# NyanCAD/Cadnip.jl

Measured on AMD Instinct MI355X. Metric: newton_iters_per_sec, higher is better.
Workload: dtype f64; 1 GPU; gf180 DFF transient 0-700 ns (synthetic sp_mos1 level-1 card, 30 MOSFETs, n=235, nnz=1090), 4096 Vdd x temp corner instances per GPU (state resident in HBM; one 8-instance workgroup per CU in flight, the rest handed out by the kernel's instance queue); step = DC init + full transient of the batch; instances_per_gpu=4096, instances_total=4096, fused=2, newton_mode=1, launches_last_step=5120, accepted_last_step=6078488, rejected_last_step=692364

## Files before the change

### cadnip.jl_amd/csrc/devices.hpp

```cpp
#pragma once
#include <hip/hip_runtime.h>
#include <math.h>
#include "../../include/cadnip_hip.h"

namespace cadnip {

#define CADNIP_CHARGE_SCALE 1e12

#ifdef CADNIP_TRACE
static __device__ unsigned long long g_trace_sum[64], g_trace_cnt[64];
static __device__ int g_trace_wave;
__shared__ unsigned long long g_trace_last;
#define CADNIP_TRACE_FINE(id) (((id) >= 8 && (id) <= 15) || (id) >= 20 || (id) == 0 || (id) == 2)
#define CADNIP_TRACE_POINT(id)                                                                          \
  do {                                                                                                  \
    if ((CADNIP_TRACE + 0 >= 2 || !CADNIP_TRACE_FINE(id)) && blockIdx.x == 0 && (int)(threadIdx.x >> 6) == g_trace_wave) { \
      unsigned long long _t = clock64();                                                                \
      if ((threadIdx.x & 63) == 0) {                                                                    \
        atomicAdd(&g_trace_sum[id], _t - g_trace_last); atomicAdd(&g_trace_cnt[id], 1ull); g_trace_last = _t; \
      }                                                                                                 \
    }                                                                                                   \
  } while (0)
#elif defined(CADNIP_MARKS)
#define CADNIP_TRACE_POINT(id) asm volatile("; @@MARK " #id)
#else
#define CADNIP_TRACE_POINT(id) do {} while (0)
#endif

__device__ __forceinline__ double dpp_pair_swap(double v) {
  int lo = __double2loint(v), hi = __double2hiint(v);
  lo = __builtin_amdgcn_update_dpp(0, lo, 0xB1, 0xF, 0xF, false);
  hi = __builtin_amdgcn_update_dpp(0, hi, 0xB1, 0xF, 0xF, false);
  return __hiloint2double(hi, lo);
}

template <class NodeT> struct DevCtxT {
  const NodeT* __restrict__ nodes;
  const int* __restrict__ ipar;
  const double* __restrict__ par;
  const double* __restrict__ wave;
  int count;
  int dev;
  double t;
  int mode;
  int initjct;
  const double* __restrict__ cache = nullptr;
};
typedef DevCtxT<int> DevCtx;

struct SlotOut {
  static constexpr bool DIRECT = false;
  __device__ __forceinline__ void Rn(int, double) const {}
  __device__ __forceinline__ double du(int) const { return 0.0; }
  double* __restrict__ g;
  double* __restrict__ c;
  double* __restrict__ b;
  int count, dev;
  __device__ __forceinline__ void G(int k, double v) const { g[k * count + dev] = v; }
  __device__ __forceinline__ void C(int k, double v) const { c[k * count + dev] = v; }
// ... 644 lines not shown
  CADNIP_TRACE_POINT(27);
}


__device__ __forceinline__ D3 m1_swap_pair(const D3& x) {
  D3 r;
  r.v = dpp_pair_swap(x.v);
#pragma unroll
  for (int i = 0; i < 3; ++i) r.p[i] = dpp_pair_swap(x.p[i]);
  return r;
}
__device__ __forceinline__ D3 m1_sel(bool c, const D3& x, const D3& y) {
  D3 r;
  r.v = c ? x.v : y.v;
#pragma unroll
  for (int i = 0; i < 3; ++i) r.p[i] = c ? x.p[i] : y.p[i];
  return r;
}


template <class Ctx, class Out>
__device__ inline void stamp_mos1_pair(const Ctx& d, const double* u, const Out& s, double* limit_w_base, int side, bool valid) {
  const double CS = CADNIP_CHARGE_SCALE;
  const bool D = side != 0;
  int nd = node_of(d, 0), ng = node_of(d, 1), ns = node_of(d, 2), nb = node_of(d, 3), ndi = node_of(d, 4), nsi = node_of(d, 5);
  int l0 = node_of(d, 6), l1 = node_of(d, 7), l2 = node_of(d, 8), l3 = node_of(d, 9);
  double Vd = volt(u, nd), Vg = volt(u, ng), Vs = volt(u, ns), Vb = volt(u, nb), Vdi = volt(u, ndi), Vsi = volt(u, nsi);
  double type = par_of(d, M1_TYPE), vt = par_of(d, M1_VT), tPhi = par_of(d, M1_TPHI), tVbi = par_of(d, M1_TVBI);
  double gamma = par_of(d, M1_GAMMA);
  const double mf = par_of(d, M1_MFACTOR), gmin_p = par_of(d, M1_GMIN), isat = par_of(d, D ? M1_DSATCUR : M1_SSATCUR);
  const double lambda = par_of(d, M1_LAMBDA), Beta = par_of(d, M1_BETA);
  const int vdep = Out::DIRECT ? d.ipar[d.dev] : 0;
  __builtin_amdgcn_sched_barrier(0);
  CADNIP_TRACE_POINT(20);
  double w_gs, w_ds, w_bs, w_bd;
  m1_limit(d, u, type, vt, tPhi, tVbi, gamma, Vg, Vb, Vdi, Vsi, l0, l1, l2, l3, w_gs, w_ds, w_bs, w_bd);
  if (limit_w_base && valid && !D) { limit_w_base[l0] = w_gs; limit_w_base[l1] = w_ds; limit_w_base[l2] = w_bs; limit_w_base[l3] = w_bd; }
  CADNIP_TRACE_POINT(21);
  {
    const double gl[6] = {1.0, -1.0, 1.0, 1.0, -1.0, 1.0};
    s.Gv(6 * side, gl);
    if constexpr (Out::DIRECT) {
      s.Rn(D ? l2 : l0, u[D ? l2 : l0] - ((D ? Vb : Vg) - Vsi));
      s.Rn(D ? l3 : l1, u[D ? l3 : l1] - (D ? Vb - Vdi : Vdi - Vsi));
    }
  }
  CADNIP_TRACE_POINT(22);
  D3 a = D3::seed(type * w_gs, 0), b = D3::seed(type * w_ds, 1), c = D3::seed(type * w_bs, 2);
  D3 dvbd = c - b, dvgd = a - b;
  const D3 vj = m1_sel(D, dvbd, c);
  const double gmin_m = gmin_p / mf;
  const double q_cb = par_of(d, D ? M1_CBD : M1_CBS), q_cbsw = par_of(d, D ? M1_CBDSW : M1_CBSSW), q_pot = par_of(d, M1_TBULKPOT), q_dep = par_of(d, M1_TDEPCAP);
  const double q_mj = par_of(d, M1_MJ), q_mjsw = par_of(d, M1_MJSW), q_f2 = par_of(d, D ? M1_F2D : M1_F2S), q_f3 = par_of(d, D ? M1_F3D : M1_F3S), q_f4 = par_of(d, D ? M1_F4D : M1_F4S);
  __builtin_amdgcn_sched_barrier(0);
  const D3 cj = m1_junction(vj, vt, gmin_m, isat), co = m1_swap_pair(cj);
  const D3 cbs = m1_sel(D, co, cj), cbd = m1_sel(D, cj, co);
  CADNIP_TRACE_POINT(23);
  int mode;
  D3 dvon, vdsat, cdrain;
  m1_channel(a, b, c, dvbd, dvgd, tPhi, tVbi, type, gamma, lambda, Beta, mode, dvon, vdsat, cdrain);
  CADNIP_TRACE_POINT(24);
  const D3 cdreq = (mode >= 0 ? type : -type) * cdrain;
  const double dW_gs = (Vg - Vsi) - w_gs, dW_ds = (Vdi - Vsi) - w_ds, dW_bs = (Vb - Vsi) - w_bs;
  const double Vk[6] = {Vd, Vg, Vs, Vb, Vdi, Vsi};
  auto row = [&](const D3& I, double (&g)[6], double& Ieq) {
    const double fa = type * I.p[0], fb = type * I.p[1], fc = type * I.p[2];
// ... 194 lines not shown
```

### cadnip.jl_amd/csrc/fused2.hip

```cpp
#include <hip/hip_runtime.h>
#include <stdio.h>
#include <stdlib.h>
#include <string.h>
#include <algorithm>
#include <vector>
#include "fused_team_kernel.hpp"

namespace cadnip {

struct F2Tables {
  std::vector<unsigned> data;
  int off[S_NSEC];
  void begin(int which) { if (data.size() & 1) data.push_back(0); off[which] = (int)data.size(); }
  void add16(const std::vector<int>& v) {
    for (size_t i = 0; i < v.size(); i += 2) data.push_back((unsigned)(v[i] & 0xFFFF) | ((i + 1 < v.size() ? (unsigned)(v[i + 1] & 0xFFFF) : 0u) << 16));
  }
  void add32(unsigned x) { data.push_back(x); }
  void add64(u64 x) { data.push_back((unsigned)x); data.push_back((unsigned)(x >> 32)); }
};

template <class Build>
static void upload_steps(StepList& L, int lu_words, Build&& build) {
  if (L.d) (void)hipFree(L.d);
  L = StepList();
// ... 109 lines not shown
}

int fused2_tables(CadnipHandle* h) {
  FusedState& S = h->f2;
  if (!h->analyzed) return CADNIP_NOTREADY;
  if (S.d_tab && !S.dirty) return CADNIP_OK;
  S.release();
  F2Tables T;
  if (!f2_prepare(h, T)) return CADNIP_BADARG;
  HIP_TRY(hipMalloc((void**)&S.d_tab, T.data.size() * sizeof(unsigned)));
  HIP_TRY(hipMemcpy(S.d_tab, T.data.data(), T.data.size() * sizeof(unsigned), hipMemcpyHostToDevice));
  for (int i = 0; i < S_NSEC; ++i) S.off[i] = T.off[i];
  S.dirty = false;
  return CADNIP_OK;
}

static int fused2_blocks(CadnipHandle* h) {
  { int rc = fused2_tables(h); if (rc) return rc; }
  FusedState& S = h->f2;
  if (S.blk_dirty || !S.d_blk) {
    F2Block hb[F2_MAX_BLOCKS];
    int nb = 0;
    for (size_t bi = 0; bi < h->blocks.size() && nb < F2_MAX_BLOCKS; ++bi) {
      auto& b = h->blocks[bi];
      if (b.count == 0) continue;
      hb[nb++] = F2Block{b.d_ipar, b.d_par, b.type, b.count, b.n_par, b.g_base, b.c_base, b.b_base, S.nodes_off[bi], b.mos1_plain ? 1 : 0, -1};
    }
    for (int i = 0; i < nb; ++i)
      for (int j = i + 1; j < nb; ++j)
        if ((hb[j].type == CADNIP_DEV_MOS1) > (hb[i].type == CADNIP_DEV_MOS1)) { F2Block tmp = hb[i]; hb[i] = hb[j]; hb[j] = tmp; }
    auto first_of = [&](int ta, int tb) { for (int i = 0; i < nb; ++i) if (hb[i].type == ta || hb[i].type == tb) return i; return -1; };
    S.rc_blk = first_of(CADNIP_DEV_CAPACITOR, CADNIP_DEV_RESISTOR);
    S.src_blk = first_of(CADNIP_DEV_VSOURCE, CADNIP_DEV_ISOURCE);
    S.lean = true;
    for (int i = 0; i < nb; ++i) {
      const int ty = hb[i].type;
      const bool heavy = ty == CADNIP_DEV_DIODE || ty == CADNIP_DEV_DIODECAP || ty == CADNIP_DEV_SIMPLEMOS || ty == CADNIP_DEV_BVSOURCE ||
                         ty == CADNIP_DEV_BISOURCE || ty == CADNIP_DEV_VA || (ty == CADNIP_DEV_MOS1 && !hb[i].mos1_plain);
      if (heavy) S.lean = false;
    }
    if (!S.steps1.d || lds_bytes(lds_sweep((size_t)0, S.lean_end - S.lean_lo, S.steps1.len, S.lu_words, h->n, 0, 8)) > LDS_BUDGET) S.lean = false;
    S.n_blk = nb;
    S.par_words = 0;
    { bool first = true;
      for (int i = 0; i < nb; ++i)
        if (hb[i].type == CADNIP_DEV_MOS1 && hb[i].mos1_plain) {
          if (!first || hb[i].count > 32) { hb[i].lds_par = S.par_words; S.par_words += hb[i].n_par * hb[i].count; }
          first = false;
        } }
    if (!S.d_blk) HIP_TRY(hipMalloc((void**)&S.d_blk, sizeof(hb)));
    HIP_TRY(hipStreamSynchronize(h->stream));
    HIP_TRY(hipMemcpy(S.d_blk, hb, sizeof(F2Block) * (size_t)nb, hipMemcpyHostToDevice));
    S.blk_dirty = false;
  }
  return CADNIP_OK;
}

F2Plan fused2_plan(CadnipHandle* h, F2Mode mode, int newton_mode) {
  F2Plan p;
  FusedState& S = h->f2;
  p.rc = CADNIP_BADARG;
  if (h->va_ext || !h->analyzed) return p;
  if (fused2_tables(h)) return p;
  int nb = 0;
  for (auto& b : h->blocks) nb += b.count > 0;
  if (nb > F2_MAX_BLOCKS || lds_bytes(lds_sweep((size_t)0, S.full_len, 0, S.lu_words, h->n, 0, 1)) > LDS_BUDGET) return p;
  if (int rc = fused2_blocks(h)) { p.rc = rc; return p; }
  const bool direct = !getenv("CADNIP_F2_NODIRECT"), lean = direct && S.lean;
  p.keep_factors = mode != F2_DC && (newton_mode || mode == F2_STEP);
  if (p.keep_factors && !lean) return p;
  p.circuit_ok = true;
  if (h->homotopy || h->spec.gshunt != 0.0 || h->spec.srcFact < 1.0) return p;
  if (S.n_cu <= 0) {
    int cu = 0;
    if (hipError_t e = hipDeviceGetAttribute(&cu, hipDeviceAttributeMultiprocessorCount, h->device)) { set_last_error("hipDeviceGetAttribute", e); p.rc = CADNIP_HIPERROR; return p; }
    S.n_cu = cu > 0 ? cu : 256;
  }
  p.var = !direct ? 2 : S.lean ? 0 : 1;
  p.tab_len = S.full_len;
  if (lean) { p.tab_lo = S.lean_lo; p.tab_len = S.lean_end - S.lean_lo; }
  if (mode != F2_DC && lean) {
    int nw = h->B <= S.n_cu ? 4 : h->B <= 2 * S.n_cu ? 2 : 0;
    if (const char* e = getenv("CADNIP_F2_TEAM")) nw = atoi(e) >= 4 ? 4 : atoi(e) >= 2 ? 2 : 0;
    if (mode == F2_STEP) nw = 4;
    const StepList& T = S.team[nw / 4];
    const size_t shmem = lds_bytes(lds_team((size_t)0, p.tab_len, nw ? T.len : 0, S.lu_words, h->n, S.par_words, nw));
    if (nw && T.d && shmem <= LDS_BUDGET) {
      const int wg_per_cu = (int)std::max<size_t>(1, std::min<size_t>(LDS_BUDGET / shmem, (size_t)(16 / nw)));
      p.nw = nw; p.steps = &T; p.shmem = shmem; p.grid = std::min(h->B, S.n_cu * wg_per_cu); p.rc = CADNIP_OK;
      return p;
    }
  }
  if (mode == F2_STEP) return p;
  if (lean) p.steps = &S.steps1;
  auto bytes = [&](int wpb) { return lds_bytes(lds_sweep((size_t)0, p.tab_len, p.steps ? p.steps->len : 0, S.lu_words, h->n, 0, wpb)); };
  int wpb = 8;
  if (const char* e = getenv("CADNIP_F2_WPB")) wpb = atoi(e) >= 8 ? 8 : atoi(e) >= 4 ? 4 : atoi(e) >= 2 ? 2 : 1;
  while (wpb > 1 && (bytes(wpb) > LDS_BUDGET || S.n_cu * (wpb / 2) >= h->B)) wpb >>= 1;
  if (bytes(wpb) > LDS_BUDGET) return p;
  const int wg_per_cu = (int)std::max<size_t>(1, std::min<size_t>(LDS_BUDGET / bytes(wpb), (size_t)(32 / wpb)));
  size_t shmem = bytes(wpb);
  if (p.steps && lds_steps_predec_ok(S.lu_words, h->n) && !getenv("CADNIP_F2_STEPS_PACKED")) {
    const size_t pd = lds_bytes(lds_sweep((size_t)0, p.tab_len, lds_sweep_desc_words(p.steps->len, true), S.lu_words, h->n, 0, wpb));
    if (pd <= LDS_BUDGET && (int)std::max<size_t>(1, std::min<size_t>(LDS_BUDGET / pd, (size_t)(32 / wpb))) == wg_per_cu) { p.step_predec = true; shmem = pd; }
  }
  p.wpb = wpb; p.shmem = shmem; p.grid = std::min((h->B + wpb - 1) / wpb, S.n_cu * wg_per_cu); p.rc = CADNIP_OK;
  return p;
}

static int launch_fused2(CadnipHandle* h, const TranArgs& t, int rounds, const F2DcOpts* dc, const F2StepOpts* step = nullptr) {
  const F2Plan p = fused2_plan(h, dc ? F2_DC : step ? F2_STEP : F2_TRAN, t.newton_mode);
  if (p.rc) return p.rc;
  ProfScope ps(h, dc ? "fused2_dc" : step ? "fused_step" : "fused2_newton");
  FusedState& S = h->f2;
  F2Args f{};
  f.n_blk = S.n_blk; f.rc_blk = S.rc_blk; f.src_blk = S.src_blk;
  f.blk = (const F2Block*)S.d_blk;
  f.wave = h->d_wave;
  f.tab = S.d_tab;
  for (int i = 0; i < S_NSEC; ++i) f.off[i] = S.off[i];
  f.tab_len = p.tab_len; f.tab_lo = p.tab_lo;
  f.n = h->n; f.nnz = h->nnz; f.nnz_lu = S.lu_words;
  f.n_pre = S.n_pre; f.n_post = S.n_post; f.nc = S.nc; f.dn0 = S.dn0; f.n_fwd = S.n_fwd;
  if (p.steps) { f.team_desc = p.steps->d; f.team_desc_len = p.steps->len; f.ts_pre = p.steps->n_steps[0]; f.ts_post = p.steps->n_steps[1]; f.ts_fwd = p.steps->n_steps[2]; }
  f.step_predec = p.step_predec ? 1 : 0;
  f.step_refresh = step ? step->refresh : 0; f.step_resid = step ? step->resid : nullptr; f.step_norm = step ? step->norm : nullptr;
  f.step_reps = step ? step->reps : 1; f.step_skip = step ? step->skip : 0;
  if (p.keep_factors) {
    const size_t need = (size_t)h->B * S.lu_words;
    if (need > S.lufac_cap) {
      if (S.d_lufac) (void)hipFree(S.d_lufac);
      S.d_lufac = nullptr; S.lufac_cap = 0;
      HIP_TRY(hipMalloc((void**)&S.d_lufac, need * sizeof(double)));
      S.lufac_cap = need;
    }
    f.lufac = S.d_lufac;
  }
  f.rounds = rounds; f.B = h->B; f.t = t; f.cold = h->d_cold;
  f.dc_mode = 1;
  if (dc) { f.dc_abstol = dc->abstol; f.dc_maxiters = dc->maxiters; f.dc_pcnr = dc->use_pcnr; f.dc_mode = dc->mode; f.dc_initjct = dc->initjct; f.dcstate = dc->dcstate; }
  if (!S.d_queue) HIP_TRY(hipMalloc((void**)&S.d_queue, sizeof(int)));
  TRY_RC(dev_zero_async(h, S.d_queue, sizeof(int)));
  f.queue = S.d_queue;
  const bool debug = getenv("CADNIP_F2_DEBUG") != nullptr;
  if (p.nw) {
    f.par_words = S.par_words;
    if (debug) fprintf(stderr, "[cadnip f2] team of %d waves: B %d n_cu %d grid %d shmem %zu rounds %d nc %d steps %d+%d / %d\n", p.nw, h->B, S.n_cu, p.grid, p.shmem, rounds, S.nc, f.ts_pre, f.ts_post, f.ts_fwd);
    if (step) TRY_RC(fteam_launch_step(std::min(h->B, S.n_cu), p.shmem, h->stream, f));
    else TRY_RC(fteam_launch(p.nw, p.grid, p.shmem, h->stream, f));
  } else {
    const size_t tab_b = (size_t)p.tab_len / 2 * 8, desc_b = (size_t)lds_sweep_desc_words(f.team_desc_len, p.step_predec) * 8;
    if (debug) fprintf(stderr, "[cadnip f2] B %d n_cu %d wpb %d grid %d shmem %zu (tables %zu, steps %zu, per instance %zu) rounds %d nc %d passes %d+%d steps %d+%d / %d (%s) variant %d\n", h->B, S.n_cu, p.wpb, p.grid, p.shmem, tab_b, desc_b, (p.shmem - tab_b - desc_b) / p.wpb, rounds, S.nc, S.n_pre, S.n_post, f.ts_pre, f.ts_post, f.ts_fwd, p.step_predec ? "pre-decoded" : "packed", p.var);
    TRY_RC(p.var == 0 ? f2_launch_variant<0>(p.wpb, dc != nullptr, p.grid, p.shmem, h->stream, f)
         : p.var == 1 ? f2_launch_variant<1>(p.wpb, dc != nullptr, p.grid, p.shmem, h->stream, f)
                      : f2_launch_variant<2>(p.wpb, dc != nullptr, p.grid, p.shmem, h->stream, f));
  }
  HIP_TRY(hipGetLastError());
  return CADNIP_OK;
}

int launch_fused2_rounds(CadnipHandle* h, const TranArgs& t, int rounds) { return launch_fused2(h, t, rounds, nullptr); }

int launch_fused_step(CadnipHandle* h, int refresh, const FusedStepIO& io) {
  TranArgs t;
  memset(&t, 0, sizeof(t));
  t.u = (double*)io.u; t.du = (double*)io.du; t.delta = io.delta; t.limit_w = h->d_limit_w; t.tcur = (double*)io.t; t.gamma = (double*)io.gamma; t.active = h->d_active; t.flags = io.flags;
  t.t = io.t_keep; t.h = io.gamma_keep;
  t.B = h->B; t.n = h->n; t.n_limits = h->n_limits;
  F2StepOpts so{refresh, io.resid, io.norm, io.reps > 0 ? io.reps : 1, io.skip};
  return launch_fused2(h, t, 1 << 30, nullptr, &so);
}

int launch_fused2_dc(CadnipHandle* h, const TranArgs& t, int rounds, double abstol, int maxiters, int use_pcnr, int mode, int initjct, int* d_dcstate) {
  F2DcOpts dc{abstol, maxiters, use_pcnr, mode, initjct, d_dcstate};
  return launch_fused2(h, t, rounds, &dc);
}

}
```

### cadnip.jl_amd/csrc/fused2_kernel.hpp

```cpp
#pragma once
#include <hip/hip_runtime.h>
#include "devices.hpp"
#include "internal.hpp"
#include "tran_ctrl.hpp"
#include "lds_layout.hpp"

namespace cadnip {

typedef unsigned short u16;
typedef unsigned long long u64;
#define NOPOS 0xFFFFu
#define F2_NCMAX 16
#define F2_JU 18
#define F2_MAX_BLOCKS 32

enum { S_GPOS = 0, S_CDESC, S_BROW, S_NZ, S_ENT, S_TERM, S_LEV, S_QINV, S_NODES, S_ROWOF, S_LOADPOS, S_NSEC };

struct F2Block {
  const int* ipar; const double* par;
  int type, count, n_par, g_base, c_base, b_base, nodes_off, mos1_plain;
  int lds_par;
};

typedef const __attribute__((address_space(4))) F2Block* F2BlockPtr;

__device__ __forceinline__ F2Block load_block(const F2Block* blk, int i) {
  F2BlockPtr q = (F2BlockPtr)blk + i;
  F2Block b;
  b.ipar = q->ipar; b.par = q->par; b.type = q->type; b.count = q->count; b.n_par = q->n_par; b.g_base = q->g_base; b.c_base = q->c_base;
  b.b_base = q->b_base; b.nodes_off = q->nodes_off; b.mos1_plain = q->mos1_plain; b.lds_par = q->lds_par;
  return b;
}

struct F2Args {
  const F2Block* blk;
  int n_blk, rc_blk;
  int src_blk;
  const double* wave;
  const unsigned* tab;
  int off[S_NSEC];
  int tab_len;
  int tab_lo;
  int n, nnz, nnz_lu, rounds, B;
  int n_pre, n_post, nc, dn0;
  int n_fwd;
  double* lufac;
  const unsigned long long* team_desc; int team_desc_len;
  int ts_pre, ts_post, ts_fwd;
  int step_predec;
  int par_words;
  int step_refresh; double *step_resid, *step_norm;
  int step_reps, step_skip;
  double dc_abstol; int dc_maxiters, dc_pcnr, dc_mode, dc_initjct; int* dcstate;
  const int* cold;
  int* queue;
  TranArgs t;
};

typedef const __attribute__((address_space(4))) F2Args* F2ArgsK;
__device__ __forceinline__ F2ArgsK kargs() {
  F2ArgsK p = (F2ArgsK)__builtin_amdgcn_kernarg_segment_ptr();
  asm volatile("" : "+s"(p));
  return p;
}
struct TranStateView {
  double *t, *h, *hprev, *hpp, *tcur, *gamma;
  int *nhist, *order, *k, *status, *bp_idx, *save_idx, *active;
  long long* cnt;
  const double *breaks, *save_t;
  int n_break, n_save;
  int newton_mode; double *mn_a0f, *mn_ss, *mn_dnp; int* mn_flags;
  int max_order; double* hp3;
};
__device__ __forceinline__ TranStateView state_view() {
  const F2ArgsK p = kargs();
  TranStateView v;
  v.t = p->t.t; v.h = p->t.h; v.hprev = p->t.hprev; v.hpp = p->t.hpp; v.tcur = p->t.tcur; v.gamma = p->t.gamma;
  v.nhist = p->t.nhist; v.order = p->t.order; v.k = p->t.k; v.status = p->t.status; v.bp_idx = p->t.bp_idx; v.save_idx = p->t.save_idx;
  v.active = p->t.active; v.cnt = p->t.cnt; v.breaks = p->t.breaks; v.save_t = p->t.save_t; v.n_break = p->t.n_break; v.n_save = p->t.n_save;
  v.newton_mode = p->t.newton_mode; v.mn_a0f = p->t.mn_a0f; v.mn_ss = p->t.mn_ss; v.mn_dnp = p->t.mn_dnp; v.mn_flags = p->t.mn_flags;
  v.max_order = p->t.max_order; v.hp3 = p->t.hp3;
  return v;
// ... 194 lines not shown
#pragma unroll
      for (int j = k + 1; j < NC; ++j) A[j] = fma(-m, readlane_f64(A[j], k), A[j]);
      if (lane > k) A[k] = m;
    }
    bc = fma(-m, readlane_f64(bc, k), bc);
  }
#pragma unroll
  for (int k = NC - 1; k >= 0; --k) {
    const double xk = readlane_f64(bc * rp[k], k);
    bc = lane == k ? xk : (lane < k ? fma(-A[k], xk, bc) : bc);
  }
  if (lane < NC) {
    W[yc0 + lane] = bc;
    if (MODE == 0 && keep) {
#pragma unroll
      for (int j = 0; j < NC; ++j) S[j] = j == lane ? rp[j] : A[j];
    }
  }
}

template <int WPB, bool DC, int VAR>
__global__ void __launch_bounds__(64 * WPB) k_fused2(F2Args f) {
  constexpr bool DIRECT = VAR != 2, LEAN = VAR == 0;
  extern __shared__ double sm[];
  const int tid = threadIdx.x, lane0 = tid & 63, w = __builtin_amdgcn_readfirstlane(tid >> 6), n = f.n;
  {
    const uint2* src = (const uint2*)(f.tab + f.tab_lo);
    uint2* dst = (uint2*)sm;
    for (int i = tid; i < f.tab_len / 2; i += 64 * WPB) dst[i] = src[i];
  }
  const TranArgs& a = f.t;
  const unsigned* tab = (const unsigned*)sm;
  const bool predec = LEAN && f.step_predec;
  const LdsSweep<double*> L = lds_sweep((double*)sm, f.tab_len, LEAN ? lds_sweep_desc_words(f.team_desc_len, predec) : 0, f.nnz_lu, n, w, WPB);
  const uint4* tdesc = (const uint4*)L.desc;
  const unsigned char* tflag = (const unsigned char*)(L.desc + (LEAN ? f.team_desc_len : 0));
  if constexpr (LEAN) {
    if (predec) {
      const uint4* src = (const uint4*)f.team_desc;
      uint4* dst = (uint4*)L.desc;
      unsigned char* fl = (unsigned char*)(L.desc + f.team_desc_len);
      for (int i = tid; i < f.team_desc_len / 2; i += 64 * WPB) {
        const uint4 d = src[i];
        const StepPredec p = lds_step_predecode(d.x, d.y, d.z, d.w, (unsigned)(f.nnz_lu + n + lane0));
        dst[i] = make_uint4(p.x, p.y, p.z, p.w);
        fl[i] = (unsigned char)p.flags;
      }
    } else {
      const uint2* src = (const uint2*)f.team_desc;
      uint2* dst = (uint2*)L.desc;
      for (int i = tid; i < f.team_desc_len; i += 64 * WPB) dst[i] = src[i];
    }
  }
  __syncthreads();
  const int nW = L.nW;
  double* W = L.W;
  double* us = L.u;
  double* betas = L.beta;
  if (lane0 == 0) { W[nW] = 0.0; W[nW + 1] = 1.0; }
  const int tlo = f.tab_lo;
  const u16* gpos = (const u16*)(tab + (f.off[S_GPOS] - tlo));
  const u64* cdesc = (const u64*)(tab + (f.off[S_CDESC] - tlo));
  const u16* brow = (const u16*)(tab + (f.off[S_BROW] - tlo));
  const u64* nzd = (const u64*)(tab + (LEAN ? 0 : f.off[S_NZ]));
  const u64* laned = (const u64*)(tab + (LEAN ? 0 : f.off[S_ENT]));
  const unsigned* term = tab + (LEAN ? 0 : f.off[S_TERM]);
  typedef const __attribute__((address_space(4))) u64* PassPtr;
// ... 56 lines not shown
  while (inst < f.B) {
    const TranStateView sv = state_view();
    if (DC) st.status = __builtin_amdgcn_readfirstlane(sv.status[inst]);
    else { st = load_state(sv, inst); make_uniform(st); }
    if (st.status == 0) { have = true; break; }
    int nx = 0;
    if (lane0 == 0) nx = atomicAdd(kargs()->queue, 1);
    inst = (int)gridDim.x * WPB + __builtin_amdgcn_readfirstlane(nx);
  }
  if (!have || budget <= 0) break;
  const size_t vo = (size_t)inst * n;
  double* lw = (DC ? f.dc_pcnr : a.use_pcnr) ? kargs()->t.limit_w + vo : nullptr;
  FusedVecs vec{us, betas, W, qinv, vo, lw};
  if (!DC) vec.load_history(n, lane0);
  {
    const F2ArgsK ka = kargs();
    const double *ug = ka->t.u + vo, *betag = ka->t.beta + vo;
    for (int i = lane0; i < n; i += 64) { us[i] = ug[i]; betas[i] = DC ? 0.0 : betag[i]; }
  }
  const bool mn = !DC && LEAN && a.newton_mode != 0;
  if (mn && (st.mflags & MN_VALID)) {
    const double* src = kargs()->lufac + (size_t)inst * f.nnz_lu;
    for (int i = lane0; i < f.nnz_lu; i += 64) W[i] = src[i];
  }
  int dc_state = 0, dc_iters = 0, dc_first = 0;
  if (DC) { dc_state = __builtin_amdgcn_readfirstlane(kargs()->dcstate[inst]); dc_first = f.dc_initjct && __builtin_amdgcn_readfirstlane(kargs()->cold[inst]); }
  double rc_val[2] = {0.0, 0.0};
  if (f.rc_blk >= 0) {
    const F2Block B = load_block(f.blk, f.rc_blk);
    const double* par = B.par + (size_t)inst * B.n_par * B.count;
#pragma unroll
    for (int q = 0; q < 2; ++q) { const int dev = lane0 + 64 * q; rc_val[q] = par[dev < B.count ? dev : 0]; }
  }
  double src_val = 0.0, src_t = 0.0;
  bool src_have = false;
  int src_seg = 0;
  for (; budget > 0; --budget) {
    int lane = lane0;
    asm volatile("" : "+v"(lane));
    CADNIP_TRACE_POINT(17);
    bool refresh = true;
    if (mn) {
      refresh = (st.mflags & MN_NEED) || !(st.mflags & MN_VALID) ||
                (st.k == 0 && (st.a0 < 0.6 * st.a0f || st.a0 * 0.6 > st.a0f || (st.mflags >> MN_SINCE_SHIFT) >= 20));
      if (refresh) { st.a0f = st.a0; st.ss = 20.0; st.mflags = MN_VALID | MN_JCUR; st.dsc = 1.0; }
      else st.dsc = st.a0 == st.a0f ? 1.0 : fast_div(2.0, 1.0 + fast_div(st.a0, st.a0f));
    }
    if (refresh) {
      for (int i = lane; i < (nW >> 1); i += 64) ((double2*)W)[i] = make_double2(0.0, 0.0);
    } else {
      for (int i = f.nnz_lu + lane; i < nW; i += 64) W[i] = 0.0;
    }
    CADNIP_WAVE_SYNC();
    CADNIP_TRACE_POINT(0);
    const double tcur = DC ? 0.0 : st.tn, a0 = DC ? 0.0 : st.a0;
    const int dmode = DC ? f.dc_mode : 1, dinit = DC ? dc_first : 0;
    const unsigned trash_w = (unsigned)(f.nnz_lu + n + lane);
    dc_first = 0;
    if constexpr (DIRECT) {
      auto at = [&](unsigned nd16) -> double { const double x = us[nd16 == 0xFFFFu ? 0u : nd16]; return nd16 == 0xFFFFu ? 0.0 : x; };
      auto dat = [&](unsigned nd16) -> double {
        const unsigned i = nd16 == 0xFFFFu ? 0u : nd16;
        const double x = a0 * us[i] + betas[i];
        return nd16 == 0xFFFFu ? 0.0 : x;
      };
      if (f.rc_blk >= 0) {
        const bool cap = rc_type == CADNIP_DEV_CAPACITOR;
        double jv[2], cur[2];
#pragma unroll
        for (int q = 0; q < 2; ++q) {
          const unsigned np = rc_nd[q] & 0xFFFFu, nn = rc_nd[q] >> 16;
          const double xp = cap ? dat(np) : at(np), xn = cap ? dat(nn) : at(nn);
          jv[q] = cap ? a0 * rc_val[q] : rc_val[q];
          cur[q] = rc_val[q] * (xp - xn);
        }
#pragma unroll
        for (int q = 0; q < 2; ++q) {
          if (q == 1 && rc_count <= 64) break;
          if (refresh) {
            atomicAdd(&W[rc_gp[q][0] & 0xFFFFu], jv[q]); atomicAdd(&W[rc_gp[q][0] >> 16], -jv[q]);
            atomicAdd(&W[rc_gp[q][1] & 0xFFFFu], -jv[q]); atomicAdd(&W[rc_gp[q][1] >> 16], jv[q]);
          }
          atomicAdd(&W[rc_row[q] & 0xFFFFu], cur[q]); atomicAdd(&W[rc_row[q] >> 16], -cur[q]);
        }
      }
      if (f.src_blk >= 0) {
        if (DC || !src_have || tcur != src_t) {
          const F2Block B = load_block(f.blk, f.src_blk);
          const double* par = B.par + (size_t)inst * B.n_par * B.count;
          LdsCtx d{nodes + B.nodes_off, B.ipar, par, f.wave, B.count, lane < B.count ? lane : 0, tcur, dmode, dinit};
          src_val = source_value(d, par_of(d, 0), par_of(d, 1), &src_seg);
          src_t = tcur; src_have = true;
        }
        if (src_type == CADNIP_DEV_VSOURCE) {
          const double ui = at(src_nd[1]), vd = at(src_nd[0] & 0xFFFFu) - at(src_nd[0] >> 16) - src_val;
          if (refresh) {
            atomicAdd(&W[src_gp[0] & 0xFFFFu], 1.0); atomicAdd(&W[src_gp[0] >> 16], -1.0);
            atomicAdd(&W[src_gp[1] & 0xFFFFu], 1.0); atomicAdd(&W[src_gp[1] >> 16], -1.0);
          }
          atomicAdd(&W[src_row[0] & 0xFFFFu], ui); atomicAdd(&W[src_row[0] >> 16], -ui);
          atomicAdd(&W[src_row[1]], vd);
        } else {
          atomicAdd(&W[src_row[0] & 0xFFFFu], -src_val); atomicAdd(&W[src_row[0] >> 16], src_val);
        }
      }
      CADNIP_TRACE_POINT(13);
    }
    for (int bi = 0; bi < f.n_blk; ++bi) {
      if (DIRECT && ((bi == f.rc_blk && rc_count <= 128) || (bi == f.src_blk && src_count <= 64))) continue;
      const F2Block B = load_block(f.blk, bi);
      const double* par = B.par + (size_t)inst * B.n_par * B.count;
      int dev0 = lane;
      if (DIRECT && bi == f.rc_blk) dev0 = lane + 128;
      if (DIRECT && bi == f.src_blk) dev0 = lane + 64;
      if (!DIRECT && bi == f.rc_blk) {
#pragma unroll
        for (int q = 0; q < 2; ++q) {
          const int dev = lane + 64 * q;
          if (dev < B.count) {
            AccumOutT<false, DIRECT> s{W, betas, a0, gpos + B.g_base, cdesc + B.c_base, brow + B.b_base, B.count, dev, 0u, us, rowof, trash_w};
            if (B.type == CADNIP_DEV_CAPACITOR) capacitance4(s, 0, rc_val[q]); else conductance4(s, 0, rc_val[q]);
            if (DIRECT) {
              const short* nd = nodes + B.nodes_off;
              const int np = nd[dev], nn = nd[B.count + dev];
              residual2(s, np, nn, B.type == CADNIP_DEV_CAPACITOR ? rc_val[q] * (s.du(np) - s.du(nn)) : rc_val[q] * (volt(us, np) - volt(us, nn)));
            }
// ... 287 lines not shown
```

### cadnip.jl_amd/csrc/internal.hpp

```cpp
#pragma once
#include <hip/hip_runtime.h>
#include <stdint.h>
#include <string>
#include <vector>
#include "../../include/cadnip_hip.h"
#include "stamp_plan.hpp"
#include "ac_hbm_plan.hpp"
#define CADNIP_MOS1_PAR_OXCAP 8
#define CADNIP_MOS1_PAR_GD 30
#define CADNIP_MOS1_PAR_GS 31

#define HIP_TRY(expr)                                                     \
  do {                                                                    \
    hipError_t _e = (expr);                                               \
    if (_e != hipSuccess) {                                               \
      cadnip::set_last_error(#expr, _e);                                  \
      return CADNIP_HIPERROR;                                             \
    }                                                                     \
  } while (0)

namespace cadnip {

void set_last_error(const char* what, hipError_t e);

// ... 43 lines not shown
  int type, count, n_nodes, n_ipar, n_par;
  int g_base, c_base, b_base, n_g, n_c, n_b;
  int* d_nodes = nullptr;
  std::vector<int> h_nodes;
  double* d_cache = nullptr; int n_cache = 0;
  int va_model = -1;
  int va_tl = 0;
  bool mos1_plain = false;
  int* d_ipar = nullptr;
  double* d_par = nullptr;
  int sp_cs = 0, sp_chunks = 0;
  struct PlanSet { StampShape shape; int *tptr = nullptr, *info = nullptr; uint4* rec = nullptr; unsigned short* rowoff = nullptr; };
  PlanSet plan[2];
};

struct ProfEntry { const char* name; double ms = 0; int64_t calls = 0; };

struct StepList { unsigned long long* d = nullptr; int len = 0, n_steps[3] = {0, 0, 0}; };

struct FusedState {
  bool dirty = true, blk_dirty = true;
  unsigned int* d_tab = nullptr;
  int off[16] = {0};
  int lu_len = 0;
  int lean_lo = 0, lean_end = 0;
  int full_len = 0;
  int lu_words = 0, nc = 0, dn0 = 0, n_pre = 0, n_post = 0, n_fwd = 0;
  std::vector<int> nodes_off;
  StepList steps1;
  StepList steps4;
  StepList team[2];
  void* d_blk = nullptr;
  int n_blk = 0, rc_blk = -1, src_blk = -1;
  int par_words = 0;
  bool lean = false;
  int* d_queue = nullptr;
  double* d_lufac = nullptr; size_t lufac_cap = 0;
  int n_cu = 0;
  int n_cu_hint() const { return n_cu > 0 ? n_cu : 256; }
  void release();
};

struct AcState {
  bool dirty = true;
  int *d_piv_rows = nullptr, *d_piv_lev_ptr = nullptr;
  unsigned char* d_nodiag = nullptr;
  double *d_bac = nullptr, *d_omega = nullptr, *d_x = nullptr, *d_berr = nullptr;
  int* d_flags = nullptr;
  size_t cap_freq = 0, cap_sys = 0;
  bool adj_ready = false;
  int *d_t_colptr = nullptr, *d_t_pos = nullptr, *d_t_row = nullptr, *d_t_diag = nullptr;
  int *d_ut_rows = nullptr, *d_ut_lev_ptr = nullptr, *d_lt_rows = nullptr, *d_lt_lev_ptr = nullptr;
  int *d_a_colptr = nullptr, *d_a_row = nullptr, *d_a_pos = nullptr;
  int n_ut_lev = 0, n_lt_lev = 0;
  int* d_pairs = nullptr;
  double *d_h = nullptr, *d_adj_x = nullptr, *d_adj_berr = nullptr;
  int* d_adj_flags = nullptr;
  size_t cap_pairs = 0, cap_adj_sys = 0, cap_adj_x = 0;
  double *d_multi_rhs = nullptr, *d_multi_h = nullptr, *d_multi_x = nullptr, *d_multi_berr = nullptr;
  int *d_multi_pairs = nullptr, *d_multi_flags = nullptr;
  size_t cap_multi_rhs = 0, cap_multi_h = 0, cap_multi_x = 0, cap_multi_pairs = 0, cap_multi_cols = 0;
  template <class F> void each_multi_buffer(F f) {
    f((void**)&d_multi_rhs); f((void**)&d_multi_h); f((void**)&d_multi_x); f((void**)&d_multi_berr); f((void**)&d_multi_pairs); f((void**)&d_multi_flags);
  }
  int memory = CADNIP_AC_LDS, max_waves = 0;
  double* d_work = nullptr; size_t cap_work = 0;
// ... 88 lines not shown
};
AcLaunch ac_launch_plan(CadnipHandle* h, long n_sys, int wpb_req);
int ac_lu_prepare(CadnipHandle* h, bool adjoint = false);
int launch_ac_lu(CadnipHandle* h, const AcLaunch& p, int n_freq, long s0, int n_sys, double gmin);
int launch_ac_adjoint(CadnipHandle* h, const AcLaunch& p, int n_freq, long s0, int n_sys, double gmin, int n_pairs, bool want_x);
int launch_ac_multi(CadnipHandle* h, const AcLaunch& p, int n_freq, long s0, int n_sys, double gmin, int n_rhs, int n_pairs, bool want_x);
int launch_ac_adjoint_multi(CadnipHandle* h, const AcLaunch& p, int n_freq, long s0, int n_sys, double gmin, int n_rhs, int n_pairs, bool want_x);
int upload_homotopy(CadnipHandle* h, const double* gshunt , const double* srcfact );
int restore_masks(CadnipHandle* h, bool cold);
int launch_calib_copy(CadnipHandle* h, long n, int reps);
#define TRY_RC(x) do { int _rc_ = (x); if (_rc_) return _rc_; } while (0)
struct MultiCopy { struct Seg { unsigned* dst; const unsigned* src; size_t words; }; Seg seg[8]; int n = 0;
  void add(void* dst, const void* src, size_t bytes) { seg[n].dst = (unsigned*)dst; seg[n].src = (const unsigned*)src; seg[n].words = bytes / 4; ++n; } };
int dev_multi_async(CadnipHandle* h, const MultiCopy& m, bool to_host);
int launch_norm2(CadnipHandle* h, const double* d_x, double* d_out);
int dev_zero_async(CadnipHandle* h, void* p, size_t bytes);
int dev_copy_async(CadnipHandle* h, void* dst, const void* src, size_t bytes, bool to_host);
int launch_negate(CadnipHandle* h, double* d_x, long n);
struct TranArgs;
int launch_fused2_rounds(CadnipHandle* h, const TranArgs& t, int rounds);
struct FusedStepIO { const double *u, *du, *gamma, *t; double *gamma_keep, *t_keep, *delta, *resid, *norm; int* flags; int reps = 1, skip = 0; };
int launch_fused_step(CadnipHandle* h, int refresh, const FusedStepIO& io);
int launch_va_setup(CadnipHandle* h, DeviceBlock& b);
int fused2_tables(CadnipHandle* h);
enum F2Mode { F2_TRAN, F2_DC, F2_STEP };
struct F2Plan {
  int rc = CADNIP_OK; bool circuit_ok = false;
  int nw = 0;
  int var = 0, wpb = 0, grid = 0; size_t shmem = 0;
  int tab_lo = 0, tab_len = 0;
  const StepList* steps = nullptr;
  bool step_predec = false;
  bool keep_factors = false;
};
F2Plan fused2_plan(CadnipHandle* h, F2Mode mode, int newton_mode);
int launch_fused2_dc(CadnipHandle* h, const TranArgs& t, int rounds, double abstol, int maxiters, int use_pcnr, int mode, int initjct, int* d_dcstate);
struct ProfScope {
  CadnipHandle* h; int idx;
  ProfScope(CadnipHandle* h, const char* name);
  ~ProfScope();
};
}
```

### cadnip.jl_amd/csrc/lds_layout.hpp

```cpp
#pragma once
#include <stddef.h>
#ifdef __HIPCC__
#include <type_traits>
#define LDS_HD __host__ __device__ __forceinline__
#else
#define LDS_HD inline
#endif

#define F2_TRASH 64
#define LDS_BUDGET ((size_t)160 * 1024)
#define LDS_OPTIN ((size_t)64 * 1024)

namespace cadnip {

LDS_HD int lds_work_words(int lu_words, int n) { return lu_words + n + F2_TRASH; }
#define LDS_CONSTS 2

struct StepPredec { unsigned x, y, z, w, flags; };
LDS_HD StepPredec lds_step_predecode(unsigned x, unsigned y, unsigned z, unsigned w, unsigned trash_word) {
  StepPredec r;
  r.x = ((x & 0x8000u) ? (x & 0x7FFFu) : trash_word) << 3 | ((x >> 16) & 0x7FFFu) << 19;
  r.y = (y & 0x7FFF7FFFu) << 3; r.z = (z & 0x7FFF7FFFu) << 3; r.w = (w & 0x7FFF7FFFu) << 3;
  const unsigned lg = (x >> 31) | ((y >> 14) & 2u) | ((y >> 29) & 4u);
  const unsigned maxlg = ((z >> 15) & 1u) | ((z >> 30) & 2u) | ((w >> 13) & 4u);
  r.flags = lg << 4 | (w >> 31) << 3 | maxlg;
  return r;
}
LDS_HD bool lds_steps_predec_ok(int lu_words, int n) { return lu_words + n + F2_TRASH + LDS_CONSTS <= 8192; }
LDS_HD int lds_sweep_desc_words(int desc_len, bool predec) { return desc_len + (predec ? desc_len / 16 : 0); }

template <class P> struct LdsSweep { P desc, W, u, beta, end; int nW, per; };
template <class P> LDS_HD LdsSweep<P> lds_sweep(P base, int tab_len, int desc_len, int lu_words, int n, int w, int wpb) {
  LdsSweep<P> L;
  L.nW = lds_work_words(lu_words, n);
  L.per = L.nW + LDS_CONSTS + 2 * n;
  L.desc = base + tab_len / 2;
  L.W = L.desc + desc_len + (size_t)w * L.per;
  L.u = L.W + L.nW + LDS_CONSTS; L.beta = L.u + n;
  L.end = L.desc + desc_len + (size_t)wpb * L.per;
  return L;
}

template <class P> struct LdsTeam { P W, red, u, beta, par, desc, priv, end; int nW; };
template <class P> LDS_HD LdsTeam<P> lds_team(P base, int tab_len, int desc_len, int lu_words, int n, int par_words, int nw) {
  LdsTeam<P> L;
  L.nW = lds_work_words(lu_words, n);
  L.W = base + tab_len / 2;
  L.red = L.W + L.nW + LDS_CONSTS; L.u = L.red + 4 * nw; L.beta = L.u + n; L.par = L.beta + n;
  L.desc = L.par + ((par_words + 1) & ~1); L.priv = L.desc + desc_len;
  L.end = L.priv + (nw ? (size_t)(nw - 1) * L.nW : 0);
  return L;
}

template <class P> struct LdsLu { P desc, W, end; int nW, per; };
template <class P> LDS_HD LdsLu<P> lds_lu(P base, int tab_len, int desc_len, int lu_words, int n, bool consts, int w, int waves) {
  LdsLu<P> L;
  L.nW = lds_work_words(lu_words, n);
  L.per = L.nW + (consts ? LDS_CONSTS : 0);
  L.desc = base + tab_len / 2;
  L.W = L.desc + desc_len + (size_t)w * L.per;
  L.end = L.desc + desc_len + (size_t)waves * L.per;
  return L;
}
template <class P> struct LdsAc { P lu, x, r, y, end; int per; };
template <class P> LDS_HD LdsAc<P> lds_ac(P base, int nnz_lu, int n, int w, int wpb) {
  LdsAc<P> L;
  L.per = 2 * (nnz_lu + 3 * n);
  L.lu = base + (size_t)w * L.per;
  L.x = L.lu + 2 * (size_t)nnz_lu; L.r = L.x + 2 * (size_t)n; L.y = L.r + 2 * (size_t)n;
  L.end = base + (size_t)wpb * L.per;
  return L;
// ... 19 lines not shown
```

Baseline: 141.4 million newton_iters/s.

## Cache source waveform segments per lane in LDS for transient sweep

Adds a per-instance LDS cache holding the current piecewise-linear segment (time bounds, endpoint values, scale) for each independent source. When every lane's time falls inside its cached segment, the value is interpolated from LDS and the global-memory source_value evaluation is skipped. On a miss the full evaluation runs and the segment is refilled from the waveform table. LDS per instance grows, but the cache is only enabled if it fits without lowering workgroups per CU, and an env var can turn it off. It also adds trace points.

```diff
diff --git a/cadnip.jl_amd/csrc/devices.hpp b/cadnip.jl_amd/csrc/devices.hpp
--- a/cadnip.jl_amd/csrc/devices.hpp
+++ b/cadnip.jl_amd/csrc/devices.hpp
@@ -11,7 +11,7 @@
 static __device__ unsigned long long g_trace_sum[64], g_trace_cnt[64];
 static __device__ int g_trace_wave;
 __shared__ unsigned long long g_trace_last;
-#define CADNIP_TRACE_FINE(id) (((id) >= 8 && (id) <= 15) || (id) >= 20 || (id) == 0 || (id) == 2)
+#define CADNIP_TRACE_FINE(id) (((id) >= 8 && (id) <= 15) || (id) >= 18 || (id) == 0 || (id) == 2)
 #define CADNIP_TRACE_POINT(id)                                                                          \
   do {                                                                                                  \
     if ((CADNIP_TRACE + 0 >= 2 || !CADNIP_TRACE_FINE(id)) && blockIdx.x == 0 && (int)(threadIdx.x >> 6) == g_trace_wave) { \
@@ -21,10 +21,13 @@
       }                                                                                                 \
     }                                                                                                   \
   } while (0)
+#define CADNIP_TRACE_USE(x) asm volatile("" ::"v"(x))
 #elif defined(CADNIP_MARKS)
 #define CADNIP_TRACE_POINT(id) asm volatile("; @@MARK " #id)
+#define CADNIP_TRACE_USE(x) do {} while (0)
 #else
 #define CADNIP_TRACE_POINT(id) do {} while (0)
+#define CADNIP_TRACE_USE(x) do {} while (0)
 #endif
 
 __device__ __forceinline__ double dpp_pair_swap(double v) {
@@ -735,6 +738,10 @@
   const double lambda = par_of(d, M1_LAMBDA), Beta = par_of(d, M1_BETA);
   const int vdep = Out::DIRECT ? d.ipar[d.dev] : 0;
   __builtin_amdgcn_sched_barrier(0);
+  CADNIP_TRACE_USE(Vd); CADNIP_TRACE_USE(Vg); CADNIP_TRACE_USE(Vs); CADNIP_TRACE_USE(Vb); CADNIP_TRACE_USE(Vdi); CADNIP_TRACE_USE(Vsi);
+  CADNIP_TRACE_POINT(18);
+  CADNIP_TRACE_USE(type);
+  CADNIP_TRACE_POINT(19);
   CADNIP_TRACE_POINT(20);
   double w_gs, w_ds, w_bs, w_bd;
   m1_limit(d, u, type, vt, tPhi, tVbi, gamma, Vg, Vb, Vdi, Vsi, l0, l1, l2, l3, w_gs, w_ds, w_bs, w_bd);
diff --git a/cadnip.jl_amd/csrc/fused2.hip b/cadnip.jl_amd/csrc/fused2.hip
--- a/cadnip.jl_amd/csrc/fused2.hip
+++ b/cadnip.jl_amd/csrc/fused2.hip
@@ -165,6 +165,7 @@
     auto first_of = [&](int ta, int tb) { for (int i = 0; i < nb; ++i) if (hb[i].type == ta || hb[i].type == tb) return i; return -1; };
     S.rc_blk = first_of(CADNIP_DEV_CAPACITOR, CADNIP_DEV_RESISTOR);
     S.src_blk = first_of(CADNIP_DEV_VSOURCE, CADNIP_DEV_ISOURCE);
+    S.src_count = S.src_blk >= 0 ? hb[S.src_blk].count : 0;
     S.lean = true;
     for (int i = 0; i < nb; ++i) {
       const int ty = hb[i].type;
@@ -188,6 +189,8 @@
   }
   return CADNIP_OK;
 }
+
+static bool env_is_zero(const char* name) { const char* e = getenv(name); return e && atoi(e) == 0; }
 
 F2Plan fused2_plan(CadnipHandle* h, F2Mode mode, int newton_mode) {
   F2Plan p;
@@ -237,6 +240,13 @@
     const size_t pd = lds_bytes(lds_sweep((size_t)0, p.tab_len, lds_sweep_desc_words(p.steps->len, true), S.lu_words, h->n, 0, wpb));
     if (pd <= LDS_BUDGET && (int)std::max<size_t>(1, std::min<size_t>(LDS_BUDGET / pd, (size_t)(32 / wpb))) == wg_per_cu) { p.step_predec = true; shmem = pd; }
   }
+  if (mode == F2_TRAN && direct && S.src_blk >= 0 && !env_is_zero("CADNIP_F2_SRC_CACHE")) {
+    const int sw = src_cache_words(S.src_count), dw = p.steps ? lds_sweep_desc_words(p.steps->len, p.step_predec) : 0;
+    if (src_cache_fits(p.tab_len, dw, S.lu_words, h->n, wpb, sw)) {
+      p.src_words = sw;
+      shmem = lds_bytes(lds_sweep((size_t)0, p.tab_len, dw, S.lu_words, h->n, 0, wpb, sw));
+    }
+  }
   p.wpb = wpb; p.shmem = shmem; p.grid = std::min((h->B + wpb - 1) / wpb, S.n_cu * wg_per_cu); p.rc = CADNIP_OK;
   return p;
 }
@@ -257,6 +267,7 @@
   f.n_pre = S.n_pre; f.n_post = S.n_post; f.nc = S.nc; f.dn0 = S.dn0; f.n_fwd = S.n_fwd;
   if (p.steps) { f.team_desc = p.steps->d; f.team_desc_len = p.steps->len; f.ts_pre = p.steps->n_steps[0]; f.ts_post = p.steps->n_steps[1]; f.ts_fwd = p.steps->n_steps[2]; }
   f.step_predec = p.step_predec ? 1 : 0;
+  f.src_words = p.src_words;
   f.step_refresh = step ? step->refresh : 0; f.step_resid = step ? step->resid : nullptr; f.step_norm = step ? step->norm : nullptr;
   f.step_reps = step ? step->reps : 1; f.step_skip = step ? step->skip : 0;
   if (p.keep_factors) {
@@ -283,7 +294,7 @@
     else TRY_RC(fteam_launch(p.nw, p.grid, p.shmem, h->stream, f));
   } else {
     const size_t tab_b = (size_t)p.tab_len / 2 * 8, desc_b = (size_t)lds_sweep_desc_words(f.team_desc_len, p.step_predec) * 8;
-    if (debug) fprintf(stderr, "[cadnip f2] B %d n_cu %d wpb %d grid %d shmem %zu (tables %zu, steps %zu, per instance %zu) rounds %d nc %d passes %d+%d steps %d+%d / %d (%s) variant %d\n", h->B, S.n_cu, p.wpb, p.grid, p.shmem, tab_b, desc_b, (p.shmem - tab_b - desc_b) / p.wpb, rounds, S.nc, S.n_pre, S.n_post, f.ts_pre, f.ts_post, f.ts_fwd, p.step_predec ? "pre-decoded" : "packed", p.var);
+    if (debug) fprintf(stderr, "[cadnip f2] B %d n_cu %d wpb %d grid %d shmem %zu (tables %zu, steps %zu, per instance %zu) rounds %d nc %d passes %d+%d steps %d+%d / %d (%s) variant %d src-cache %d\n", h->B, S.n_cu, p.wpb, p.grid, p.shmem, tab_b, desc_b, (p.shmem - tab_b - desc_b) / p.wpb, rounds, S.nc, S.n_pre, S.n_post, f.ts_pre, f.ts_post, f.ts_fwd, p.step_predec ? "pre-decoded" : "packed", p.var, p.src_words);
     TRY_RC(p.var == 0 ? f2_launch_variant<0>(p.wpb, dc != nullptr, p.grid, p.shmem, h->stream, f)
          : p.var == 1 ? f2_launch_variant<1>(p.wpb, dc != nullptr, p.grid, p.shmem, h->stream, f)
                       : f2_launch_variant<2>(p.wpb, dc != nullptr, p.grid, p.shmem, h->stream, f));
diff --git a/cadnip.jl_amd/csrc/fused2_kernel.hpp b/cadnip.jl_amd/csrc/fused2_kernel.hpp
--- a/cadnip.jl_amd/csrc/fused2_kernel.hpp
+++ b/cadnip.jl_amd/csrc/fused2_kernel.hpp
@@ -4,6 +4,7 @@
 #include "internal.hpp"
 #include "tran_ctrl.hpp"
 #include "lds_layout.hpp"
+#include "src_cache.hpp"
 
 namespace cadnip {
 
@@ -48,6 +49,7 @@
   const unsigned long long* team_desc; int team_desc_len;
   int ts_pre, ts_post, ts_fwd;
   int step_predec;
+  int src_words;
   int par_words;
   int step_refresh; double *step_resid, *step_norm;
   int step_reps, step_skip;
@@ -308,7 +310,7 @@
   const TranArgs& a = f.t;
   const unsigned* tab = (const unsigned*)sm;
   const bool predec = LEAN && f.step_predec;
-  const LdsSweep<double*> L = lds_sweep((double*)sm, f.tab_len, LEAN ? lds_sweep_desc_words(f.team_desc_len, predec) : 0, f.nnz_lu, n, w, WPB);
+  const LdsSweep<double*> L = lds_sweep((double*)sm, f.tab_len, LEAN ? lds_sweep_desc_words(f.team_desc_len, predec) : 0, f.nnz_lu, n, w, WPB, f.src_words);
   const uint4* tdesc = (const uint4*)L.desc;
   const unsigned char* tflag = (const unsigned char*)(L.desc + (LEAN ? f.team_desc_len : 0));
   if constexpr (LEAN) {
@@ -431,6 +433,14 @@
 #pragma unroll
     for (int q = 0; q < 2; ++q) { const int dev = lane0 + 64 * q; rc_val[q] = par[dev < B.count ? dev : 0]; }
   }
+  auto sc_on = [&]() -> bool { return !DC && DIRECT && kargs()->src_words > 0; };
+  if (sc_on()) {
+    const F2Block B = load_block(f.blk, f.src_blk);
+    const int cl = src_cache_lanes(B.count);
+    int ln = lane0;
+    asm volatile("" : "+v"(ln));
+    if (ln < cl) src_seg_store(L.src, cl, ln, src_seg_fill(B.ipar[ln], (B.par + (size_t)inst * B.n_par * B.count)[ln]));
+  }
   double src_val = 0.0, src_t = 0.0;
   bool src_have = false;
   int src_seg = 0;
@@ -483,14 +493,39 @@
           atomicAdd(&W[rc_row[q] & 0xFFFFu], cur[q]); atomicAdd(&W[rc_row[q] >> 16], -cur[q]);
         }
       }
+      CADNIP_TRACE_POINT(14);
       if (f.src_blk >= 0) {
         if (DC || !src_have || tcur != src_t) {
-          const F2Block B = load_block(f.blk, f.src_blk);
-          const double* par = B.par + (size_t)inst * B.n_par * B.count;
-          LdsCtx d{nodes + B.nodes_off, B.ipar, par, f.wave, B.count, lane < B.count ? lane : 0, tcur, dmode, dinit};
-          src_val = source_value(d, par_of(d, 0), par_of(d, 1), &src_seg);
+          const int cl = src_cache_lanes(src_count);
+          const bool sc = sc_on();
+          int miss = 1;
+          double cv = 0.0;
+          if (sc) {
+            const SrcSeg e = src_seg_load((const double*)L.src, cl, lane < cl ? lane : 0);
+            miss = src_seg_hit(e, tcur) ? 0 : 1;
+            cv = src_seg_value(e, tcur);
+          }
+          if (wave_any(miss)) {
+            const F2Block B = load_block(f.blk, f.src_blk);
+            const double* par = B.par + (size_t)inst * B.n_par * B.count;
+            LdsCtx d{nodes + B.nodes_off, B.ipar, par, f.wave, B.count, lane < B.count ? lane : 0, tcur, dmode, dinit};
+            src_val = source_value(d, par_of(d, 0), par_of(d, 1), &src_seg);
+          } else src_val = cv;
+          if (sc_on() && miss && lane < cl) {
+            const F2ArgsK ka = kargs();
+            const F2Block B = load_block(ka->blk, ka->src_blk);
+            SrcSeg r = src_seg_never();
+            if (B.ipar[lane] == 1) {
+              const int len = B.ipar[2 * B.count + lane];
+              const double* wv = ka->wave + B.ipar[B.count + lane];
+              r = src_seg_refill(1, wv, wv + len, len, src_seg, (B.par + (size_t)inst * B.n_par * B.count)[B.count + lane]);
+            }
+            src_seg_store(L.src, cl, lane, r);
+          }
           src_t = tcur; src_have = true;
         }
+        CADNIP_TRACE_USE(src_val);
+        CADNIP_TRACE_POINT(15);
         if (src_type == CADNIP_DEV_VSOURCE) {
           const double ui = at(src_nd[1]), vd = at(src_nd[0] & 0xFFFFu) - at(src_nd[0] >> 16) - src_val;
           if (refresh) {
diff --git a/cadnip.jl_amd/csrc/internal.hpp b/cadnip.jl_amd/csrc/internal.hpp
--- a/cadnip.jl_amd/csrc/internal.hpp
+++ b/cadnip.jl_amd/csrc/internal.hpp
@@ -99,6 +99,7 @@
   StepList team[2];
   void* d_blk = nullptr;
   int n_blk = 0, rc_blk = -1, src_blk = -1;
+  int src_count = 0;
   int par_words = 0;
   bool lean = false;
   int* d_queue = nullptr;
@@ -253,6 +254,7 @@
   const StepList* steps = nullptr;
   bool step_predec = false;
   bool keep_factors = false;
+  int src_words = 0;
 };
 F2Plan fused2_plan(CadnipHandle* h, F2Mode mode, int newton_mode);
 int launch_fused2_dc(CadnipHandle* h, const TranArgs& t, int rounds, double abstol, int maxiters, int use_pcnr, int mode, int initjct, int* d_dcstate);
diff --git a/cadnip.jl_amd/csrc/lds_layout.hpp b/cadnip.jl_amd/csrc/lds_layout.hpp
--- a/cadnip.jl_amd/csrc/lds_layout.hpp
+++ b/cadnip.jl_amd/csrc/lds_layout.hpp
@@ -29,14 +29,14 @@
 LDS_HD bool lds_steps_predec_ok(int lu_words, int n) { return lu_words + n + F2_TRASH + LDS_CONSTS <= 8192; }
 LDS_HD int lds_sweep_desc_words(int desc_len, bool predec) { return desc_len + (predec ? desc_len / 16 : 0); }
 
-template <class P> struct LdsSweep { P desc, W, u, beta, end; int nW, per; };
-template <class P> LDS_HD LdsSweep<P> lds_sweep(P base, int tab_len, int desc_len, int lu_words, int n, int w, int wpb) {
+template <class P> struct LdsSweep { P desc, W, u, beta, end; int nW, per; P src; };
+template <class P> LDS_HD LdsSweep<P> lds_sweep(P base, int tab_len, int desc_len, int lu_words, int n, int w, int wpb, int src_words = 0) {
   LdsSweep<P> L;
   L.nW = lds_work_words(lu_words, n);
-  L.per = L.nW + LDS_CONSTS + 2 * n;
+  L.per = L.nW + LDS_CONSTS + 2 * n + src_words;
   L.desc = base + tab_len / 2;
   L.W = L.desc + desc_len + (size_t)w * L.per;
-  L.u = L.W + L.nW + LDS_CONSTS; L.beta = L.u + n;
+  L.u = L.W + L.nW + LDS_CONSTS; L.beta = L.u + n; L.src = L.beta + n;
   L.end = L.desc + desc_len + (size_t)wpb * L.per;
   return L;
 }
diff --git a/cadnip.jl_amd/csrc/src_cache.hpp b/cadnip.jl_amd/csrc/src_cache.hpp
--- /dev/null
+++ b/cadnip.jl_amd/csrc/src_cache.hpp
@@ -0,0 +1,56 @@
+#pragma once
+#include "lds_layout.hpp"
+
+namespace cadnip {
+
+#define SRC_CACHE_FIELDS 5
+#define SRC_CACHE_LANES 64
+
+struct SrcSeg { double t_lo, t_hi, y_lo, y_hi, scale; };
+
+LDS_HD int src_cache_lanes(int src_count) { return src_count < SRC_CACHE_LANES ? (src_count > 0 ? src_count : 0) : SRC_CACHE_LANES; }
+LDS_HD int src_cache_words(int src_count) { return (SRC_CACHE_FIELDS * src_cache_lanes(src_count) + 1) & ~1; }
+
+LDS_HD SrcSeg src_seg_never() { SrcSeg e; e.t_lo = __builtin_inf(); e.t_hi = __builtin_inf(); e.y_lo = 0.0; e.y_hi = 0.0; e.scale = 1.0; return e; }
+LDS_HD SrcSeg src_seg_make(double t_lo, double t_hi, double y_lo, double y_hi, double scale) {
+  SrcSeg e; e.t_lo = t_lo; e.t_hi = t_hi; e.y_lo = y_lo; e.y_hi = y_hi; e.scale = scale; return e;
+}
+LDS_HD SrcSeg src_seg_fill(int kind, double dc) {
+  return kind == 0 ? src_seg_make(-__builtin_inf(), __builtin_inf(), dc, dc, 1.0) : src_seg_never();
+}
+LDS_HD bool src_seg_hit(const SrcSeg& e, double t) { return e.t_lo < t && t < e.t_hi; }
+LDS_HD double src_seg_value(const SrcSeg& e, double t) {
+  double v;
+  if (e.y_lo == e.y_hi) v = e.y_hi;
+  else v = e.y_lo + (t - e.t_lo) * ((e.y_hi - e.y_lo) / (e.t_hi - e.t_lo));
+  return e.scale * v;
+}
+LDS_HD SrcSeg src_seg_refill(int kind, const double* ts, const double* ys, int len, int i, double scale) {
+  if (kind != 1 || len < 1) return src_seg_never();
+  if (i <= 1) return src_seg_make(-__builtin_inf(), ts[0], ys[0], ys[0], scale);
+  if (i > len) return src_seg_make(ts[len - 1], __builtin_inf(), ys[len - 1], ys[len - 1], scale);
+  const double t_lo = ts[i - 2], t_hi = ts[i - 1];
+  if (!(t_lo < t_hi)) return src_seg_never();
+  return src_seg_make(t_lo, t_hi, ys[i - 2], ys[i - 1], scale);
+}
+
+template <class P> LDS_HD SrcSeg src_seg_load(P base, int count, int lane) {
+  return src_seg_make(base[lane], base[count + lane], base[2 * count + lane], base[3 * count + lane], base[4 * count + lane]);
+}
+template <class P> LDS_HD void src_seg_store(P base, int count, int lane, const SrcSeg& e) {
+  base[lane] = e.t_lo; base[count + lane] = e.t_hi; base[2 * count + lane] = e.y_lo; base[3 * count + lane] = e.y_hi; base[4 * count + lane] = e.scale;
+}
+
+LDS_HD int sweep_wg_per_cu(size_t bytes, int wpb) {
+  size_t k = bytes ? LDS_BUDGET / bytes : 0, cap = (size_t)(32 / wpb);
+  if (k > cap) k = cap;
+  return k < 1 ? 1 : (int)k;
+}
+LDS_HD bool src_cache_fits(int tab_len, int desc_words, int lu_words, int n, int wpb, int src_words) {
+  if (src_words <= 0) return false;
+  const size_t without = lds_bytes(lds_sweep((size_t)0, tab_len, desc_words, lu_words, n, 0, wpb));
+  const size_t with = lds_bytes(lds_sweep((size_t)0, tab_len, desc_words, lu_words, n, 0, wpb, src_words));
+  return with <= LDS_BUDGET && sweep_wg_per_cu(with, wpb) == sweep_wg_per_cu(without, wpb);
+}
+
+}
```

After: 145.6 million newton_iters/s (median of 6 runs). +2.9%, better.
